# agrif/unnamed-rust-sdr

Measured on AMD Instinct MI355X. Metric: complex Msamples/sec through 255-tap FIR, 1/2/4/8 MI355X; % HBM roofline, higher is better.
Workload: dtype f32

## Files before the change

### unnamed-rust-sdr_amd/csrc/fir_mxh.hip

```cpp
#include <algorithm>
#include <climits>
#include <cstdlib>
#include <type_traits>
#include <utility>

#include "fir_kernels.hpp"

namespace sdrgpu {

namespace {

typedef _Float16 f16x8 __attribute__((ext_vector_type(8)));
typedef unsigned u32x4 __attribute__((ext_vector_type(4)));
typedef float f32x4 __attribute__((ext_vector_type(4)));

constexpr int kWaves = 8;
constexpr int kBlock = 64 * kWaves;
constexpr int kCs1 = 4;
constexpr int kCs2 = 2;
constexpr int cs_of(int D) { return D == 1 ? kCs1 : (D == 2 ? kCs2 : 1); }
constexpr int kRunTiles = 2;
constexpr int kRunTilesU8 = 8;
constexpr int kStagePerChunk = 4;
constexpr int kNonFinite = 1 << 16;

template <int NCH, int D = 4, int CS = 1>
struct GeoH {
    static constexpr int TO = 256 * CS;
    static constexpr int TI = TO * D;
    static constexpr int HR = 32 * NCH - 16 * D;
    static constexpr int H = (HR + 127) / 128 * 128;
    static constexpr int OFF = H - HR;
    static constexpr int R = H + 2 * TI;
    static constexpr int PLB = 2 * R;
    static constexpr int WODD = 2 * TI;
    static constexpr int WAVE = 4 * PLB;
    static constexpr int NG = TI / 128;
    static constexpr int NH = H / 128;
    static_assert(HR > 0 && (D == 1 || ((D == 4 || D == 2) && OFF == 0)), "geometry");
    static_assert(TI >= H && (D == 1 || TI % 1024 == 0), "ring");
    static_assert(kWaves * WAVE <= 160 * 1024, "LDS");
};

struct MxhParams {
    const float2* in;
    const unsigned* in_u8;
    long ld_in, n_in;
    const float2* hist;
    float2* hist_next;
    const float2* dummy;
    long n_out;
    int K;
    int delta;
    int sh;
    const float* taps;
    const u32x4* frags;
    float2* out;
    long ld_out;
    long tpc, spc, seg_tiles, units;
    int ftiles;
    int oblk;
    int vec_out;
    int blocked;
};

__device__ __forceinline__ f32x4 mfma(const u32x4& a, const u32x4& b, f32x4 c) {
    return __builtin_amdgcn_mfma_f32_16x16x32_f16(__builtin_bit_cast(f16x8, a),
                                                  __builtin_bit_cast(f16x8, b), c, 0, 0, 0);
}

__device__ __forceinline__ unsigned pk_rtz(float a, float b) {
    return __builtin_bit_cast(unsigned, __builtin_amdgcn_cvt_pkrtz(a, b));
}

__device__ __forceinline__ float lo_f(unsigned u) {
    return (float)__builtin_bit_cast(_Float16, (unsigned short)(u & 0xffffu));
}
__device__ __forceinline__ float hi_f(unsigned u) {
    return (float)__builtin_bit_cast(_Float16, (unsigned short)(u >> 16));
}

__device__ __forceinline__ void split2(float a, float b, unsigned& hi, unsigned& lo) {
    hi = pk_rtz(a, b);
    lo = pk_rtz(a - lo_f(hi), b - hi_f(hi));
}

__device__ __forceinline__ int sigma(int v) {
    return v < 4 ? 2 * v : (v >= 12 ? 2 * v - 16 : 2 * v - 7);
}

__device__ __forceinline__ float2 fetch1(const float2* in, const float2* hist, long j, long n_in,
                                         int K) {
    const bool inb = (j >= 0) & (j < n_in);
    const bool inh = (j < 0) & (j >= -(long)(K - 1));
    const float2 xa = in[inb ? j : 0];
    const float2 xb = hist[inh ? j + (K - 1) : 0];
    return inb ? xa : (inh ? xb : make_float2(0.f, 0.f));
}

__device__ __forceinline__ float4 fetch_pair(const float2* in, const float2* hist, long j,
                                             long n_in, int K) {
    const float2 a = fetch1(in, hist, j, n_in, K), b = fetch1(in, hist, j + 1, n_in, K);
    return make_float4(a.x, a.y, b.x, b.y);
}

__device__ __forceinline__ float2 u8_iq(unsigned short w) {
    return make_float2(((float)(w & 0xffu) - 128.0f) / 128.0f, ((float)(w >> 8) - 128.0f) / 128.0f);
}
__device__ __forceinline__ unsigned iq_u8(float2 v) {
    return (unsigned)(v.x * 128.0f + 128.0f) | ((unsigned)(v.y * 128.0f + 128.0f) << 8);
}
__device__ __forceinline__ unsigned fetch_pair_u8(const unsigned short* in, const float2* hist,
                                                  long j, long n_in, int K) {
    unsigned w = 0;
#pragma unroll
    for (int e = 0; e < 2; ++e) {
        const long q = j + e;
        const bool inb = (q >= 0) & (q < n_in);
        const bool inh = (q < 0) & (q >= -(long)(K - 1));
        const unsigned a = in[inb ? q : 0];
        const unsigned b = iq_u8(hist[inh ? q + (K - 1) : 0]);
        w |= (inb ? a : (inh ? b : 0x8080u)) << (16 * e);
    }
    return w;
}
template <int PLB>
__device__ __forceinline__ void put_pair_u8(char* lds, int a, unsigned w) {
    const float r0 = (float)(w & 0xffu) - 128.f, i0 = (float)((w >> 8) & 0xffu) - 128.f;
    const float r1 = (float)((w >> 16) & 0xffu) - 128.f, i1 = (float)(w >> 24) - 128.f;
    *reinterpret_cast<unsigned*>(lds + a) = pk_rtz(r0, r1);
    *reinterpret_cast<unsigned*>(lds + a + 2 * PLB) = pk_rtz(i0, i1);
}

__device__ __forceinline__ void st32(char* lds, int a, unsigned v) {
    *reinterpret_cast<unsigned*>(lds + a) = v;
}

template <int PLB>
__device__ __forceinline__ void put_pair(char* lds, int a, const float4& f, float sc) {
    unsigned h, l;
    split2(f.x * sc, f.z * sc, h, l);
    st32(lds, a, h);
    st32(lds, a + PLB, l);
    split2(f.y * sc, f.w * sc, h, l);
    st32(lds, a + 2 * PLB, h);
    st32(lds, a + 3 * PLB, l);
}

__device__ __forceinline__ float absmax4(float m, const float4& f) {
    auto mx = [](float a, float b) { return __builtin_elementwise_maximum(a, b); };
    return mx(mx(mx(mx(m, fabsf(f.x)), fabsf(f.y)), fabsf(f.z)), fabsf(f.w));
}

template <int CTRL>
__device__ __forceinline__ unsigned dpp_umax(unsigned x) {
    const unsigned y = (unsigned)__builtin_amdgcn_mov_dpp((int)x, CTRL, 0xf, 0xf, true);
    return x > y ? x : y;
}
__device__ __forceinline__ int wave_scale(float m) {
    unsigned x = __float_as_uint(m);
    x = dpp_umax<0xB1>(x);
    x = dpp_umax<0x4E>(x);
    x = dpp_umax<0x141>(x);
    x = dpp_umax<0x140>(x);
    const unsigned a = __builtin_amdgcn_readlane(x, 0), b = __builtin_amdgcn_readlane(x, 16);
    const unsigned c = __builtin_amdgcn_readlane(x, 32), d = __builtin_amdgcn_readlane(x, 48);
    const unsigned ab = a > b ? a : b, cd = c > d ? c : d;
    const int e = (int)((ab > cd ? ab : cd) >> 23);
    const int s = 141 - e;
    return e == 255 ? kNonFinite : (s < -126 ? -126 : (s > 126 ? 126 : s));
}

__device__ __forceinline__ float mul_add_vop2(float acc, float x, float h) {
    float p, r;
    asm("v_mul_f32 %0, %1, %2" : "=v"(p) : "v"(x), "v"(h));
    asm("v_add_f32 %0, %1, %2" : "=v"(r) : "v"(acc), "v"(p));
    return r;
}

template <int D, int CS>
__device__ __forceinline__ void exact_tile(const MxhParams& p, long ch, int tile, int sv, int g) {
#pragma clang fp contract(off)
    const int K = p.K;
    const float2* __restrict__ in = p.in + ch * p.ld_in;
    const float2* __restrict__ hist = p.hist + ch * (long)(K - 1);
    float2* __restrict__ out = p.out + ch * p.ld_out;
    const long i0 = D - 1 - p.delta;
#pragma unroll 1
    for (int o = 0; o < 4 * CS; ++o) {
        {
            const long m = (long)tile * (256 * CS) + 256 * (o >> 2) + 16 * sv + 4 * g + (o & 3);
            if (m >= p.n_out) continue;
            const long gi = i0 + (long)D * m;
            float ar = 0.f, ai = 0.f;
            if (gi - (K - 1) >= 0 && gi < p.n_in) {
                const float2* __restrict__ xp = in + gi;
                const int kb = K & ~15;
#pragma unroll 1
                for (int k = 0; k < kb; k += 16) {
                    float2 xv[16];
                    float hk[16];
#pragma unroll
                    for (int u = 0; u < 16; ++u) {
                        xv[u] = xp[-(k + u)];
                        hk[u] = p.taps[k + u];
                    }
#pragma unroll
                    for (int u = 0; u < 16; ++u) {
                        ar = mul_add_vop2(ar, xv[u].x, hk[u]);
                        ai = mul_add_vop2(ai, xv[u].y, hk[u]);
                    }
                }
#pragma unroll 1
                for (int k = kb; k < K; ++k) {
                    const float2 xv = xp[-k];
                    const float hk = p.taps[k];
                    ar = mul_add_vop2(ar, xv.x, hk);
                    ai = mul_add_vop2(ai, xv.y, hk);
                }
            } else {
#pragma unroll 1
                for (int k = 0; k < K; ++k) {
                    const float2 xv = fetch1(in, hist, gi - k, p.n_in, K);
                    const float hk = p.taps[k];
                    ar = mul_add_vop2(ar, xv.x, hk);
                    ai = mul_add_vop2(ai, xv.y, hk);
                }
            }
            out[m] = make_float2(ar, ai);
        }
    }
}

__device__ __forceinline__ float exp2i(int s) { return __builtin_amdgcn_ldexpf(1.0f, s); }

template <int NCH, int D>
__global__ __launch_bounds__(64) void tap_frag_kernel(const float* __restrict__ taps, int K, int sh,
                                                      u32x4* __restrict__ tab) {
    constexpr int HR = GeoH<NCH, D, cs_of(D)>::HR;
    const int lane = threadIdx.x, delta = blockIdx.x;
    const int g = lane >> 4, v = lane & 15;
    const float tsc = exp2i(sh);
    u32x4* __restrict__ th = tab + (size_t)delta * (2 * NCH * 64);
#pragma unroll
    for (int c = 0; c < NCH; ++c) {
        u32x4 ah, al;
#pragma unroll
        for (int jj = 0; jj < 4; ++jj) {
            unsigned hw = 0, lw = 0;
#pragma unroll
            for (int e = 0; e < 2; ++e) {
                const int pidx = 32 * c + 8 * g + 2 * jj + e;
                const int k = D * v + D - 1 - delta + HR - pidx;
                const bool ok = (k >= 0) & (k < K);
                const float hk = taps[ok ? k : 0];
                const float hs = ok ? hk * tsc : 0.f;
                const _Float16 h16 = (_Float16)hs;
                const _Float16 l16 = (_Float16)(hs - (float)h16);
                hw |= (unsigned)__builtin_bit_cast(unsigned short, h16) << (16 * e);
                lw |= (unsigned)__builtin_bit_cast(unsigned short, l16) << (16 * e);
            }
            ah[jj] = hw;
            al[jj] = lw;
        }
        th[c * 64 + lane] = ah;
        th[(NCH + c) * 64 + lane] = al;
    }
}

template <int NCH, bool U8 = false, int D = 4, int CS = 1>
__global__ __launch_bounds__(kBlock) __attribute__((amdgpu_waves_per_eu(2, 2)))
void fir_mxh_kernel(MxhParams p) {
    using Raw = std::conditional_t<U8, unsigned, float4>;
    using G = GeoH<NCH, D, CS>;
    constexpr int H = G::H, PLB = G::PLB, NH = G::NH, NG = G::NG;
    constexpr int TI = G::TI;
    extern __shared__ __attribute__((aligned(16))) char smem[];

    claim_simd_half();
    const int lane = threadIdx.x & 63;
    const int wv = __builtin_amdgcn_readfirstlane(threadIdx.x >> 6);
    if (wv >= kWaves / 2) __builtin_amdgcn_s_setprio(1);
    const long wave = (long)blockIdx.x * kWaves + wv;
    const long nwaves = (long)gridDim.x * kWaves;
    const int g = lane >> 4, v = lane & 15;
    const int K = p.K;
    const int base = wv * G::WAVE;

    u32x4 ah[NCH], al[NCH];
    const int sv = D == 4 ? sigma(v) : v;
    int rb[NCH];
    int wb0;
    auto ramp_setup = [&]() {
#pragma unroll
        for (int c = 0; c < NCH; ++c) {
            ah[c] = p.frags[c * 64 + lane];
            al[c] = p.frags[(NCH + c) * 64 + lane];
        }
#pragma unroll
        for (int c = 0; c < NCH; ++c) {
            if constexpr (D == 4) {
                const int r = sv + (c >> 1);
                rb[c] = base + 128 * r + 16 * ((4 * (c & 1) + g) ^ ((r >> 1) & 7));
            } else if constexpr (D == 2) {
                const int r = v + c;
                rb[c] = base + 64 * r + 16 * (g ^ ((r >> 1) & 3));
            } else {
                rb[c] = base + 2 * (G::OFF + 16 * sv + 32 * c + 8 * g);
            }
        }
        wb0 = D == 4   ? base + 128 * (lane >> 5) + 4 * (lane & 3) + 16 * ((lane >> 2) & 7)
              : D == 2 ? base + 64 * (lane >> 4) + 4 * (lane & 3) + 16 * (((lane >> 2) & 3) ^ (lane >> 5))
                       : base + 4 * lane;
    };

    struct Cur {
        int u, t, ch, tu, nt;
        int ok;
    };
    const int units = (int)p.units, spc = (int)p.spc, segt = (int)p.seg_tiles, tpc = (int)p.tpc;
    const int ust = p.blocked ? kWaves : (int)nwaves;
    const int ub1 = p.blocked ? (int)(((long)blockIdx.x + 1) * p.units / gridDim.x) : units;
    auto seek = [&](Cur& c, int u) {
        c.u = u;
        c.t = 0;
        c.ok = u < ub1;
        if constexpr (D == 4 && !U8) {
            c.ch = c.ok && spc < units ? u / spc : 0;
        } else {
            c.ch = c.ok ? u / spc : 0;
        }
        c.tu = (u - c.ch * spc) * segt;
        c.nt = c.ok ? std::min(segt, tpc - c.tu) : 0;
        if (c.ok && c.nt <= 0) c.ok = false;
    };
    auto adv = [&](Cur& c) {
        if (!c.ok) return;
        if (++c.t >= c.nt) seek(c, c.u + ust);
    };
    const long n_in = p.n_in;
    auto tile_j0 = [&](const Cur& c) { return (long)TI * (c.tu + c.t); };
    auto tile_fast = [&](const Cur& c) { return c.tu + c.t < p.ftiles; };
    auto fetch = [&](const Cur& c, long j) -> Raw {
        const float2* hist = p.hist + c.ch * (long)(K - 1);
        if constexpr (U8)
            return fetch_pair_u8(reinterpret_cast<const unsigned short*>(p.in_u8) + c.ch * p.ld_in, hist, j,
                                 n_in, K);
        else
            return fetch_pair(p.in + c.ch * p.ld_in, hist, j, n_in, K);
    };
    auto put = [&](int a, const Raw& w, float sc) {
        if constexpr (U8) put_pair_u8<PLB>(smem, a, w);
        else put_pair<PLB>(smem, a, w, sc);
    };
    auto ldx = [&](const Cur& c, long j, auto nt_c) -> Raw {
        constexpr bool NT = decltype(nt_c)::value;
        if constexpr (U8) {
            const unsigned* q = p.in_u8 + c.ch * (p.ld_in / 2) + (j >> 1);
            return NT ? __builtin_nontemporal_load(q) : *q;
        } else {
            const f32x4* q = reinterpret_cast<const f32x4*>(p.in + c.ch * p.ld_in + j);
            const f32x4 r = NT ? __builtin_nontemporal_load(q) : *q;
            return make_float4(r[0], r[1], r[2], r[3]);
        }
    };
    auto load_tile = [&](Raw (&dst)[NG], const Cur& c) {
        const long j0 = tile_j0(c);
        if (tile_fast(c)) {
#pragma unroll
            for (int k = 0; k < NG; ++k) dst[k] = ldx(c, j0 + 128 * k + 2 * lane, std::true_type());
        } else {
            asm volatile("" ::: "memory");
#pragma unroll
            for (int k = 0; k < NG; ++k) dst[k] = fetch(c, j0 + 128 * k + 2 * lane);
        }
    };
    auto load_hist = [&](Raw (&dst)[NH], const Cur& c) {
        const long j = tile_j0(c) - H;
        const int tile = c.tu + c.t;
        if (tile >= 1 && tile <= p.ftiles) {
#pragma unroll
            for (int k = 0; k < NH; ++k) dst[k] = ldx(c, j + 128 * k + 2 * lane, std::false_type());
        } else {
            asm volatile("" ::: "memory");
#pragma unroll
            for (int k = 0; k < NH; ++k) dst[k] = fetch(c, j + 128 * k + 2 * lane);
        }
    };
    auto window_scale = [&](const Raw (&nx)[NG], const Raw (&hr)[NH]) -> int {
        if constexpr (U8) {
            return 7;
        } else {
            float m = 0.f;
#pragma unroll
            for (int k = 0; k < NG; ++k) m = absmax4(m, nx[k]);
#pragma unroll
            for (int k = 0; k < NH; ++k) m = absmax4(m, hr[k]);
            return wave_scale(m);
        }
    };
    auto hist_addr = [&](int k) {
        if constexpr (D == 4) return (wb0 ^ (16 * (k & 7))) + 256 * k;
        else if constexpr (D == 2) return (wb0 ^ (32 * (k & 1))) + 256 * k;
        else return wb0 + 256 * k;
    };
    auto new_addr = [&](int k) {
        if constexpr (D == 4) return (wb0 ^ (16 * ((H / 128 + k) & 7))) + 128 * (H / 64 + 2 * k);
        else if constexpr (D == 2) return (wb0 ^ (32 * ((H / 128 + k) & 1))) + 2 * H + 256 * k;
        else return wb0 + 2 * H + 256 * k;
    };
    auto roll_hist = [&](Raw (&hr)[NH], const Raw (&tile)[NG]) {
        Raw nh[NH];
#pragma unroll
        for (int i = 0; i < NH; ++i) nh[i] = NG + i < NH ? hr[(NG + i) % NH] : tile[(NG + i - NH) % NG];
#pragma unroll
        for (int i = 0; i < NH; ++i) hr[i] = nh[i];
    };

    const bool ev = (v & 1) == 0;
    const unsigned om = 8u * (16 * sv + 4 * g), omp = 8u * (16 * (D == 4 ? sigma(v ^ 1) : (v ^ 1)) + 4 * g);
    const unsigned ob1 = ev ? om : omp + 16, ob2 = ev ? omp : om + 16;

    static_assert(NG <= 8 && 2 * NG > 8, "one raw tile in flight");
    static_assert(NG > NH, "an even window's last NH groups come from keep[]");
    Cur cm, st, ld;
    const int first_unit = p.blocked ? (int)((long)blockIdx.x * p.units / gridDim.x) + wv : (int)wave;
    int nf_tiles = 0;
    seek(cm, first_unit);
    if (cm.ok) {
        Raw nx[NG], hr[NH];
        load_hist(hr, cm);
        load_tile(nx, cm);
        ramp_setup();
        st = cm;
        adv(st);
        const bool st_run = st.ok && st.t == 0;
        int s_cur = window_scale(nx, hr);
        {
            const float sc = exp2i(s_cur);
#pragma unroll
            for (int k = 0; k < NH; ++k) put(hist_addr(k), hr[k], sc);
            if (st.ok && tile_fast(st)) {
                if (st_run) load_hist(hr, st);
                const long j1 = tile_j0(st);
                Raw keep[NH];
#pragma unroll
                for (int k = 0; k < NG; ++k) {
                    put(new_addr(k), nx[k], sc);
                    if (k >= NG - NH) keep[k - (NG - NH)] = nx[k];
                    nx[k] = ldx(st, j1 + 128 * k + 2 * lane, std::true_type());
                }
                if (!st_run) {
                    Raw tile[NG];
#pragma unroll
                    for (int k = 0; k < NG; ++k) tile[k] = keep[k < NG - NH ? 0 : k - (NG - NH)];
                    roll_hist(hr, tile);
                }
            } else {
#pragma unroll
                for (int k = 0; k < NG; ++k) put(new_addr(k), nx[k], sc);
                if (st_run) load_hist(hr, st);
                else roll_hist(hr, nx);
                if (st.ok) load_tile(nx, st);
            }
        }
        ld = st;
        adv(ld);

        auto body = [&](auto tau_c) {
            constexpr int TAU = decltype(tau_c)::value;
            constexpr int P = 1 - TAU;
            constexpr int WN = P * G::WODD;
            const bool fast2 = ld.ok && tile_fast(ld);
            const bool ld_run = ld.ok && ld.t == 0;
            const long j2 = tile_j0(ld);
            const float2* src2 = fast2 ? p.in + ld.ch * p.ld_in + j2 : p.dummy;
            const unsigned* src2u = fast2 ? p.in_u8 + ld.ch * (p.ld_in / 2) + (j2 >> 1)
                                          : reinterpret_cast<const unsigned*>(p.dummy);
            const int s_fresh = window_scale(nx, hr);
            const int dsc = s_fresh - s_cur;
            const bool keep_scale = P == 1 && st.t > 0 && dsc >= -1 && dsc <= 7;
            const int s_next = keep_scale ? s_cur : s_fresh;
            const bool hist_late = P == 1 && !keep_scale;
            const float scn = exp2i(s_next);
            constexpr int NK = NG < NH ? NG : NH;
            Raw keep[NK];
            f32x4 cr[CS], ci[CS];
#pragma unroll
            for (int j = 0; j < CS; ++j) {
                cr[j] = f32x4{0.f, 0.f, 0.f, 0.f};
                ci[j] = f32x4{0.f, 0.f, 0.f, 0.f};
            }
            u32x4 fb[2][4];
            auto read_frags = [&](u32x4 (&f)[4], int c, int j) {
                const int a = rb[c] + TAU * G::WODD + j * 2 * 256 * D;
#pragma unroll
                for (int q = 0; q < 4; ++q)
                    if (!U8 || (q & 1) == 0)
                        f[q] = *reinterpret_cast<const u32x4*>(smem + a + q * PLB);
            };
            read_frags(fb[0], 0, 0);
            constexpr bool kShare = D == 1 && 32 * (NCH - 1) == 256;
#pragma unroll
            for (int i = 0; i < CS * NCH; ++i) {
                const int j = i / NCH, c = i % NCH;
                {
                    const int ni = i + 1;
                    const bool reuse = kShare && ni % NCH == 0;
                    if (ni < CS * NCH && !reuse)
                        read_frags(fb[(kShare ? ni - ni / NCH : ni) & 1], ni % NCH, ni / NCH);
                    __builtin_amdgcn_sched_barrier(0);
                    const u32x4(&f)[4] = fb[(kShare ? i - j : i) & 1];
                    cr[j] = mfma(al[c], f[0], cr[j]);
                    ci[j] = mfma(al[c], f[2], ci[j]);
                    if (!U8) {
                        cr[j] = mfma(ah[c], f[1], cr[j]);
                        ci[j] = mfma(ah[c], f[3], ci[j]);
                    }
                    cr[j] = mfma(ah[c], f[0], cr[j]);
                    ci[j] = mfma(ah[c], f[2], ci[j]);
                }
                if (i == 0) {
                    if (P == 0) {
#pragma unroll
                        for (int k = 0; k < NH; ++k) put(WN + hist_addr(k), hr[k], scn);
                    }
                    if (ld_run && !hist_late) load_hist(hr, ld);
                }
#pragma unroll
                for (int k = 0; k < NG; ++k) {
                    if ((k / kStagePerChunk < CS * NCH - 1 ? k / kStagePerChunk : CS * NCH - 1) != i) continue;
                    if (P == 1 || k < NG - NH) put(WN + new_addr(k), nx[k], scn);
                    if (k >= NG - NH) keep[k - (NG > NH ? NG - NH : 0)] = nx[k];
                    if constexpr (U8) {
                        nx[k] = __builtin_nontemporal_load(src2u + 64 * k + lane);
                    } else {
                        const f32x4 r = __builtin_nontemporal_load(
                            reinterpret_cast<const f32x4*>(src2 + 128 * k + 2 * lane));
                        nx[k] = make_float4(r[0], r[1], r[2], r[3]);
                    }
                }
            }
            if constexpr (P == 0) {
#pragma unroll
                for (int k = NG - NH; k < NG; ++k) put(WN + new_addr(k), keep[k - (NG - NH)], scn);
            } else {
                if (hist_late) {
#pragma unroll
                    for (int k = 0; k < NH; ++k) put(WN + hist_addr(k), hr[k], scn);
                    if (ld_run) load_hist(hr, ld);
                }
            }
            if (!ld_run) {
                Raw tile[NG];
#pragma unroll
                for (int k = 0; k < NG; ++k) tile[k] = keep[k < (NG > NH ? NG - NH : 0) ? 0 : k - (NG > NH ? NG - NH : 0)];
                roll_hist(hr, tile);
            }
            if (!fast2 && ld.ok) load_tile(nx, ld);
            const int so = -(s_cur + p.sh);
            const int tile = cm.tu + cm.t;
            if (!U8 && s_cur == kNonFinite) {
                ++nf_tiles;
            } else {
                float2* __restrict__ out = p.out + cm.ch * p.ld_out;
                char* __restrict__ outt = reinterpret_cast<char*>(out + (long)tile * G::TO);
#pragma unroll
                for (int j = 0; j < CS; ++j) {
                    float yr[4], yi[4];
#pragma unroll
                    for (int i = 0; i < 4; ++i) {
                        yr[i] = __builtin_amdgcn_ldexpf(cr[j][i], so);
                        yi[i] = __builtin_amdgcn_ldexpf(ci[j][i], so);
                    }
                    if (p.vec_out && tile * CS + j < p.oblk) {
                        const f32x4 y0 = {yr[0], yi[0], yr[1], yi[1]};
                        const f32x4 y1 = {yr[2], yi[2], yr[3], yi[3]};
                        f32x4 rx;
#pragma unroll
                        for (int q = 0; q < 4; ++q)
                            rx[q] = __int_as_float(__builtin_amdgcn_mov_dpp(
                                __float_as_int(ev ? y1[q] : y0[q]), 0xB1, 0xf, 0xf, false));
                        __builtin_nontemporal_store(ev ? y0 : rx, reinterpret_cast<f32x4*>(outt + (ob1 + 2048u * j)));
                        __builtin_nontemporal_store(ev ? rx : y1, reinterpret_cast<f32x4*>(outt + (ob2 + 2048u * j)));
                    } else {
                        const long m = (long)tile * G::TO + 256 * j + 16 * sv + 4 * g;
#pragma unroll
                        for (int i = 0; i < 4; ++i)
                            if (m + i < p.n_out) out[m + i] = make_float2(yr[i], yi[i]);
                    }
                }
            }
            s_cur = s_next;
            cm = st;
            st = ld;
            adv(ld);
        };
        while (cm.ok) {
            body(std::integral_constant<int, 0>());
            if (!cm.ok) break;
            body(std::integral_constant<int, 1>());
        }
    }
    if constexpr (!U8) {
        if (nf_tiles > 0) {
            Cur c;
            seek(c, first_unit);
            while (c.ok) {
                const long j0 = tile_j0(c) - H;
                bool bad = false;
                for (int q = lane; q < H + TI; q += 64) {
                    const float2 xv = fetch1(p.in + c.ch * p.ld_in, p.hist + c.ch * (long)(K - 1),
                                             j0 + q, n_in, K);
                    bad |= !(__builtin_isfinite(xv.x) && __builtin_isfinite(xv.y));
                }
                if (__builtin_amdgcn_ballot_w64(bad) != 0) exact_tile<D, CS>(p, c.ch, c.tu + c.t, sv, g);
                adv(c);
            }
        }
    }

    if (p.hist_next) {
        const long nch = p.units / p.spc;
        for (long j = (long)blockIdx.x * kBlock + threadIdx.x; j < nch * (K - 1);
             j += (long)gridDim.x * kBlock) {
            const long ch = j / (K - 1), jj = j - ch * (K - 1);
            const float2* inc = p.in + ch * p.ld_in;
            const float2* hic = p.hist + ch * (long)(K - 1);
            const long gidx = p.n_in - (long)(K - 1) + jj;
            if constexpr (U8) {
                const unsigned short* inb = reinterpret_cast<const unsigned short*>(p.in_u8) + ch * p.ld_in;
                p.hist_next[j] = gidx >= 0 ? u8_iq(inb[gidx]) : hic[gidx + (K - 1)];
            } else {
                p.hist_next[j] = gidx >= 0 ? inc[gidx] : hic[gidx + (K - 1)];
            }
        }
    }
}

int mxh_nch(int K, int D) {
    if (D == 4) {
        const int need = (K + 63 + 31) / 32;
        return need <= 6 ? 6 : (need <= 10 ? 10 : 0);
    }
    if (D == 1) {
        const int need = (K + 15 + 31) / 32;
        return need <= 5 ? 5 : (need <= 9 ? 9 : 0);
    }
    if (D == 2) {
        const int need = (K + 31 + 31) / 32;
        return need <= 5 ? 5 : (need <= 9 ? 9 : 0);
    }
    return 0;
}

}

size_t fir_mxh_dummy_bytes() { return 1024 * sizeof(float2); }

int fir_mxh_shape_ok(int sample_kind, int tap_kind, int K, int D) {
    if (tap_kind != SDRGPU_F32 || K < 1) return 0;
    if (sample_kind == SDRGPU_CU8) return D == 4 && mxh_nch(K, 4) > 0;
    return sample_kind == SDRGPU_C64 && mxh_nch(K, D) > 0;
}

int fir_mxh_supported(const FirParams& fp) {
    const bool u8 = fp.sample_kind == SDRGPU_CU8;
    if ((!u8 && fp.sample_kind != SDRGPU_C64) || fp.tap_kind != SDRGPU_F32) return 0;
    if (!(fp.D == 4 || ((fp.D == 1 || fp.D == 2) && !u8))) return 0;
    if (fp.K < 1 || mxh_nch(fp.K, fp.D) == 0) return 0;
    if (fp.i0 < 0 || fp.i0 >= fp.D) return 0;
    const uintptr_t align = u8 ? 3 : 15;
    if ((reinterpret_cast<uintptr_t>(fp.in) & align) != 0 || (fp.nch > 1 && (fp.ld_in & 1)))
        return 0;
    return 1;
}

size_t fir_mxh_frag_bytes(int K, int D) {
    const int NCH = K >= 1 ? mxh_nch(K, D) : 0;
    return (size_t)D * 2 * NCH * 64 * sizeof(u32x4);
}

int fir_mxh_frag_build(const float* d_taps, int K, int D, int tap_scale_exp, void* d_frags,
                       hipStream_t s) {
    const int NCH = K >= 1 ? mxh_nch(K, D) : 0;
    if (NCH == 0 || !d_taps || !d_frags) return SDRGPU_ERR_UNSUPPORTED;
#define SDRGPU_MXH_FRAGS(CC, DD)                                                               \
    if (D == DD && NCH == CC) {                                                                \
        hipLaunchKernelGGL((tap_frag_kernel<CC, DD>), dim3(DD), dim3(64), 0, s, d_taps, K,     \
                           tap_scale_exp, static_cast<u32x4*>(d_frags));                       \
        SDRGPU_LAUNCH_CHECK();                                                                 \
        return SDRGPU_OK;                                                                      \
    }
    SDRGPU_MXH_FRAGS(10, 4)
    SDRGPU_MXH_FRAGS(6, 4)
    SDRGPU_MXH_FRAGS(9, 1)
    SDRGPU_MXH_FRAGS(5, 1)
    SDRGPU_MXH_FRAGS(9, 2)
    SDRGPU_MXH_FRAGS(5, 2)
#undef SDRGPU_MXH_FRAGS
    return SDRGPU_ERR_UNSUPPORTED;
}

int fir_mxh_launch(const FirParams& fp, const float* d_taps, int tap_scale_exp,
                   const void* d_frags, const void* d_dummy, int cus, hipStream_t s) {
    if (!fir_mxh_supported(fp) || !d_dummy || !d_frags) return SDRGPU_ERR_UNSUPPORTED;
    const int D = fp.D;
    const int NCH = mxh_nch(fp.K, D);
    MxhParams p;
    const bool u8 = fp.sample_kind == SDRGPU_CU8;
    p.in = static_cast<const float2*>(fp.in);
    p.in_u8 = static_cast<const unsigned*>(fp.in);
    p.ld_in = fp.ld_in;
    p.n_in = fp.n_in;
    p.hist = static_cast<const float2*>(fp.hist);
    p.hist_next = fp.K > 1 ? static_cast<float2*>(fp.hist_next) : nullptr;
    p.dummy = static_cast<const float2*>(d_dummy);
    p.n_out = fp.n_out;
    p.K = fp.K;
    p.delta = (int)(D - 1 - fp.i0);
    p.sh = tap_scale_exp;
    p.taps = d_taps;
    p.frags = static_cast<const u32x4*>(d_frags) + (size_t)p.delta * (2 * NCH * 64);
    p.out = static_cast<float2*>(fp.out);
    p.ld_out = fp.ld_out;
    p.vec_out = ((reinterpret_cast<uintptr_t>(fp.out) & 15) == 0 &&
                 (fp.nch == 1 || !(fp.ld_out & 1)))
                    ? 1
                    : 0;
    const long nch = fp.nch;
    const int cs = cs_of(D);
    p.tpc = ceil_div(std::max(0L, fp.n_out), 256L * cs);
    const long W = (long)kWaves * cus;
    const int run = D == 4 ? (u8 ? kRunTilesU8 : kRunTiles) : (D == 2 ? kRunTiles : 0);
    long spc = nch >= W ? 1 : ceil_div(W, nch);
    spc = std::max(1L, std::min(spc, p.tpc));
    p.seg_tiles = std::max(1L, ceil_div(p.tpc, spc));
    if (run > 0) p.seg_tiles = std::max(1L, std::min<long>(run, p.tpc));
    p.spc = std::max(1L, ceil_div(p.tpc, p.seg_tiles));
    p.units = nch * p.spc;
    p.blocked = run > 0 && u8;
    const long TI = 256L * cs * D;
    p.ftiles = (int)std::min<long>(fp.n_in / TI, INT_MAX);
    p.oblk = (int)std::min<long>(std::max(0L, fp.n_out) / 256, INT_MAX);
    if (p.units >= INT_MAX - 8L * cus || p.tpc >= INT_MAX) return SDRGPU_ERR_UNSUPPORTED;
    const long blocks = std::max(1L, std::min((long)cus, ceil_div(p.units, kWaves)));
#define SDRGPU_MXH_GO(CC, U, DD, CS)                                                           \
    hipLaunchKernelGGL((fir_mxh_kernel<CC, U, DD, CS>), dim3(blocks), dim3(kBlock),            \
                       (size_t)kWaves * (GeoH<CC, DD, CS>::WAVE), s, p)
#define SDRGPU_MXH_CASE(CC)                                                                    \
    if (D == 4 && NCH == CC) {                                                                 \
        if (u8) SDRGPU_MXH_GO(CC, true, 4, 1);                                                 \
        else SDRGPU_MXH_GO(CC, false, 4, 1);                                                   \
        SDRGPU_LAUNCH_CHECK();                                                                 \
        return SDRGPU_OK;                                                                      \
    }
#define SDRGPU_MXH_CASE1(CC)                                                                   \
    if (D == 1 && NCH == CC) {                                                                 \
        SDRGPU_MXH_GO(CC, false, 1, kCs1);                                                     \
        SDRGPU_LAUNCH_CHECK();                                                                 \
        return SDRGPU_OK;                                                                      \
    }
#define SDRGPU_MXH_CASE2(CC)                                                                   \
    if (D == 2 && NCH == CC) {                                                                 \
        SDRGPU_MXH_GO(CC, false, 2, kCs2);                                                     \
        SDRGPU_LAUNCH_CHECK();                                                                 \
        return SDRGPU_OK;                                                                      \
    }
    SDRGPU_MXH_CASE(10)
    SDRGPU_MXH_CASE(6)
    SDRGPU_MXH_CASE1(9)
    SDRGPU_MXH_CASE1(5)
    SDRGPU_MXH_CASE2(9)
    SDRGPU_MXH_CASE2(5)
#undef SDRGPU_MXH_CASE
#undef SDRGPU_MXH_CASE1
#undef SDRGPU_MXH_CASE2
#undef SDRGPU_MXH_GO
    return SDRGPU_ERR_UNSUPPORTED;
}

}
```

Before: 631,200.

## Pair real/imag columns in MFMA fragments to halve LDS fragment reads

For float input with decimation 4 or 1, the kernel now has half the lanes read real-plane and half read imag-plane fragments. Each fragment read of two registers then feeds both the real and the (shifted) imaginary accumulators, and staging is interleaved into the new chunk loop. An extra IMO pad offsets the imaginary planes in LDS to avoid bank conflicts. Outputs are re-paired with a DPP row shuffle before the vector stores. This is meant to cut LDS read traffic, at the cost of more MFMA iterations (NCH+PSH chunks), extra select and DPP work in the epilogue, and more complex indexing.

```diff
diff --git a/unnamed-rust-sdr_amd/csrc/fir_mxh.hip b/unnamed-rust-sdr_amd/csrc/fir_mxh.hip
--- a/unnamed-rust-sdr_amd/csrc/fir_mxh.hip
+++ b/unnamed-rust-sdr_amd/csrc/fir_mxh.hip
@@ -24,7 +24,7 @@
 constexpr int kStagePerChunk = 4;
 constexpr int kNonFinite = 1 << 16;
 
-template <int NCH, int D = 4, int CS = 1>
+template <int NCH, int D = 4, int CS = 1, int IMO = 0>
 struct GeoH {
     static constexpr int TO = 256 * CS;
     static constexpr int TI = TO * D;
@@ -33,14 +33,21 @@
     static constexpr int OFF = H - HR;
     static constexpr int R = H + 2 * TI;
     static constexpr int PLB = 2 * R;
+    static constexpr int IMOFF = IMO;
     static constexpr int WODD = 2 * TI;
-    static constexpr int WAVE = 4 * PLB;
+    static constexpr int WAVE = 4 * PLB + IMO;
     static constexpr int NG = TI / 128;
     static constexpr int NH = H / 128;
     static_assert(HR > 0 && (D == 1 || ((D == 4 || D == 2) && OFF == 0)), "geometry");
     static_assert(TI >= H && (D == 1 || TI % 1024 == 0), "ring");
-    static_assert(kWaves * WAVE <= 160 * 1024, "LDS");
+    static_assert(kWaves * WAVE <= 160 * 1024 && IMO % 128 == 0, "LDS");
 };
+
+constexpr bool pair_cols(bool U8, int D) { return D == 4 && !U8; }
+constexpr bool pair_cols1(bool U8, int D) { return D == 1 && !U8; }
+constexpr int pair_imo(bool U8, int D) { return pair_cols(U8, D) ? 128 : 0; }
+template <int NCH, bool U8, int D, int CS>
+using GeoK = GeoH<NCH, D, CS, pair_imo(U8, D)>;
 
 struct MxhParams {
     const float2* in;
@@ -136,15 +143,15 @@
     *reinterpret_cast<unsigned*>(lds + a) = v;
 }
 
-template <int PLB>
+template <int PLB, int IMO>
 __device__ __forceinline__ void put_pair(char* lds, int a, const float4& f, float sc) {
     unsigned h, l;
     split2(f.x * sc, f.z * sc, h, l);
     st32(lds, a, h);
     st32(lds, a + PLB, l);
     split2(f.y * sc, f.w * sc, h, l);
-    st32(lds, a + 2 * PLB, h);
-    st32(lds, a + 3 * PLB, l);
+    st32(lds, a + 2 * PLB + IMO, h);
+    st32(lds, a + 3 * PLB + IMO, l);
 }
 
 __device__ __forceinline__ float absmax4(float m, const float4& f) {
@@ -272,9 +279,15 @@
 __global__ __launch_bounds__(kBlock) __attribute__((amdgpu_waves_per_eu(2, 2)))
 void fir_mxh_kernel(MxhParams p) {
     using Raw = std::conditional_t<U8, unsigned, float4>;
-    using G = GeoH<NCH, D, CS>;
+    using G = GeoK<NCH, U8, D, CS>;
     constexpr int H = G::H, PLB = G::PLB, NH = G::NH, NG = G::NG;
     constexpr int TI = G::TI;
+    constexpr bool PAIR = pair_cols(U8, D);
+    constexpr bool PAIR1 = pair_cols1(U8, D);
+    constexpr bool PAIRS = PAIR || PAIR1;
+    constexpr int PSH = PAIR ? 2 : 4;
+    constexpr int SETCH = 8;
+    constexpr int NRD = PAIR ? NCH + 2 : NCH;
     extern __shared__ __attribute__((aligned(16))) char smem[];
 
     claim_simd_half();
@@ -289,7 +302,8 @@
 
     u32x4 ah[NCH], al[NCH];
     const int sv = D == 4 ? sigma(v) : v;
-    int rb[NCH];
+    const int pw = v & 7, pim = ((v + 4) >> 3) & 1;
+    int rb[NRD];
     int wb0;
     auto ramp_setup = [&]() {
 #pragma unroll
@@ -298,8 +312,13 @@
             al[c] = p.frags[(NCH + c) * 64 + lane];
         }
 #pragma unroll
-        for (int c = 0; c < NCH; ++c) {
-            if constexpr (D == 4) {
+        for (int c = 0; c < NRD; ++c) {
+            if constexpr (PAIR) {
+                const int r = 2 * pw + (c >> 1);
+                rb[c] = base + pim * (2 * PLB + G::IMOFF) + 128 * r + 16 * ((4 * (c & 1) + g) ^ ((pw + (c >> 2)) & 7));
+            } else if constexpr (PAIR1) {
+                rb[c] = base + pim * 2 * PLB + 2 * (G::OFF + 16 * pw + 32 * c + 8 * g);
+            } else if constexpr (D == 4) {
                 const int r = sv + (c >> 1);
                 rb[c] = base + 128 * r + 16 * ((4 * (c & 1) + g) ^ ((r >> 1) & 7));
             } else if constexpr (D == 2) {
@@ -351,7 +370,7 @@
     };
     auto put = [&](int a, const Raw& w, float sc) {
         if constexpr (U8) put_pair_u8<PLB>(smem, a, w);
-        else put_pair<PLB>(smem, a, w, sc);
+        else put_pair<PLB, G::IMOFF>(smem, a, w, sc);
     };
     auto ldx = [&](const Cur& c, long j, auto nt_c) -> Raw {
         constexpr bool NT = decltype(nt_c)::value;
@@ -499,18 +518,65 @@
                     if (!U8 || (q & 1) == 0)
                         f[q] = *reinterpret_cast<const u32x4*>(smem + a + q * PLB);
             };
-            read_frags(fb[0], 0, 0);
-            constexpr bool kShare = D == 1 && 32 * (NCH - 1) == 256;
-#pragma unroll
-            for (int i = 0; i < CS * NCH; ++i) {
-                const int j = i / NCH, c = i % NCH;
-                {
+            auto read_pair = [&](u32x4 (&f)[4], int c) {
+                const int a = (PAIR1 ? rb[0] + 64 * c : rb[c]) + TAU * G::WODD;
+                f[0] = *reinterpret_cast<const u32x4*>(smem + a);
+                f[1] = *reinterpret_cast<const u32x4*>(smem + a + PLB);
+            };
+            if constexpr (PAIRS) read_pair(fb[0], 0);
+            else read_frags(fb[0], 0, 0);
+            if constexpr (PAIRS) {
+                constexpr int NIT = (CS - 1) * SETCH + NCH + PSH;
+                constexpr int NST = (NG + kStagePerChunk - 1) / kStagePerChunk;
+                static_assert(NST < NIT, "staging chunks");
+                auto stage = [&](int i) __attribute__((always_inline)) {
+                    if (i == 0) {
+                        if (P == 0) {
+#pragma unroll
+                            for (int k = 0; k < NH; ++k) put(WN + hist_addr(k), hr[k], scn);
+                        }
+                        if (ld_run && !hist_late) load_hist(hr, ld);
+                    }
+#pragma unroll
+                    for (int k = 0; k < NG; ++k) {
+                        if (k / kStagePerChunk != i) continue;
+                        if (P == 1 || k < NG - NH) put(WN + new_addr(k), nx[k], scn);
+                        if (k >= NG - NH) keep[k - (NG - NH)] = nx[k];
+                        const f32x4 r = __builtin_nontemporal_load(
+                            reinterpret_cast<const f32x4*>(src2 + 128 * k + 2 * lane));
+                        nx[k] = make_float4(r[0], r[1], r[2], r[3]);
+                    }
+                };
+                auto chunk = [&](int i) __attribute__((always_inline)) {
+                    if (i + 1 < NIT) read_pair(fb[(i + 1) & 1], i + 1);
+                    __builtin_amdgcn_sched_barrier(0);
+                    const u32x4(&f)[4] = fb[i & 1];
+#pragma unroll
+                    for (int m = 0; m < 3; ++m) {
+#pragma unroll
+                        for (int j = 0; j < CS; ++j) {
+                            const int c = i - SETCH * j;
+                            if (c >= 0 && c < NCH) cr[j] = mfma(m == 0 ? al[c] : ah[c], f[m == 1], cr[j]);
+                            if (c >= PSH && c < NCH + PSH)
+                                ci[j] = mfma(m == 0 ? al[c - PSH] : ah[c - PSH], f[m == 1], ci[j]);
+                        }
+                    }
+                };
+#pragma unroll
+                for (int i = 0; i < NST; ++i) {
+                    chunk(i);
+                    stage(i);
+                }
+#pragma unroll
+                for (int i = NST; i < NIT; ++i) chunk(i);
+            } else {
+#pragma unroll
+                for (int i = 0; i < CS * NCH; ++i) {
+                    const int j = i / NCH, c = i % NCH;
                     const int ni = i + 1;
-                    const bool reuse = kShare && ni % NCH == 0;
-                    if (ni < CS * NCH && !reuse)
-                        read_frags(fb[(kShare ? ni - ni / NCH : ni) & 1], ni % NCH, ni / NCH);
+                    if (ni < CS * NCH) read_frags(fb[ni & 1], ni % NCH, ni / NCH);
                     __builtin_amdgcn_sched_barrier(0);
-                    const u32x4(&f)[4] = fb[(kShare ? i - j : i) & 1];
+                    const u32x4(&f)[4] = fb[i & 1];
                     cr[j] = mfma(al[c], f[0], cr[j]);
                     ci[j] = mfma(al[c], f[2], ci[j]);
                     if (!U8) {
@@ -519,25 +585,25 @@
                     }
                     cr[j] = mfma(ah[c], f[0], cr[j]);
                     ci[j] = mfma(ah[c], f[2], ci[j]);
-                }
-                if (i == 0) {
-                    if (P == 0) {
-#pragma unroll
-                        for (int k = 0; k < NH; ++k) put(WN + hist_addr(k), hr[k], scn);
-                    }
-                    if (ld_run && !hist_late) load_hist(hr, ld);
-                }
-#pragma unroll
-                for (int k = 0; k < NG; ++k) {
-                    if ((k / kStagePerChunk < CS * NCH - 1 ? k / kStagePerChunk : CS * NCH - 1) != i) continue;
-                    if (P == 1 || k < NG - NH) put(WN + new_addr(k), nx[k], scn);
-                    if (k >= NG - NH) keep[k - (NG > NH ? NG - NH : 0)] = nx[k];
-                    if constexpr (U8) {
-                        nx[k] = __builtin_nontemporal_load(src2u + 64 * k + lane);
-                    } else {
-                        const f32x4 r = __builtin_nontemporal_load(
-                            reinterpret_cast<const f32x4*>(src2 + 128 * k + 2 * lane));
-                        nx[k] = make_float4(r[0], r[1], r[2], r[3]);
+                    if (i == 0) {
+                        if (P == 0) {
+#pragma unroll
+                            for (int k = 0; k < NH; ++k) put(WN + hist_addr(k), hr[k], scn);
+                        }
+                        if (ld_run && !hist_late) load_hist(hr, ld);
+                    }
+#pragma unroll
+                    for (int k = 0; k < NG; ++k) {
+                        if ((k / kStagePerChunk < CS * NCH - 1 ? k / kStagePerChunk : CS * NCH - 1) != i) continue;
+                        if (P == 1 || k < NG - NH) put(WN + new_addr(k), nx[k], scn);
+                        if (k >= NG - NH) keep[k - (NG > NH ? NG - NH : 0)] = nx[k];
+                        if constexpr (U8) {
+                            nx[k] = __builtin_nontemporal_load(src2u + 64 * k + lane);
+                        } else {
+                            const f32x4 r = __builtin_nontemporal_load(
+                                reinterpret_cast<const f32x4*>(src2 + 128 * k + 2 * lane));
+                            nx[k] = make_float4(r[0], r[1], r[2], r[3]);
+                        }
                     }
                 }
             }
@@ -565,29 +631,66 @@
             } else {
                 float2* __restrict__ out = p.out + cm.ch * p.ld_out;
                 char* __restrict__ outt = reinterpret_cast<char*>(out + (long)tile * G::TO);
-#pragma unroll
-                for (int j = 0; j < CS; ++j) {
-                    float yr[4], yi[4];
-#pragma unroll
-                    for (int i = 0; i < 4; ++i) {
-                        yr[i] = __builtin_amdgcn_ldexpf(cr[j][i], so);
-                        yi[i] = __builtin_amdgcn_ldexpf(ci[j][i], so);
-                    }
-                    if (p.vec_out && tile * CS + j < p.oblk) {
-                        const f32x4 y0 = {yr[0], yi[0], yr[1], yi[1]};
-                        const f32x4 y1 = {yr[2], yi[2], yr[3], yi[3]};
+                if constexpr (PAIRS) {
+                    constexpr unsigned PB = PAIR ? 16 : 128;
+                    const unsigned po = (PAIR ? 32 : 16) * pw + 4 * g + 2 * pim;
+#pragma unroll
+                    for (int j = 0; j < CS; ++j) {
+                        float a0[4], a1[4];
+#pragma unroll
+                        for (int i = 0; i < 4; ++i) {
+                            a0[i] = __builtin_amdgcn_ldexpf(cr[j][i], so);
+                            a1[i] = __builtin_amdgcn_ldexpf(ci[j][i], so);
+                        }
+                        const bool im = pim != 0;
+                        const f32x4 tx = {im ? a0[0] : a0[2], im ? a0[1] : a0[3], im ? a1[0] : a1[2],
+                                          im ? a1[1] : a1[3]};
                         f32x4 rx;
 #pragma unroll
                         for (int q = 0; q < 4; ++q)
-                            rx[q] = __int_as_float(__builtin_amdgcn_mov_dpp(
-                                __float_as_int(ev ? y1[q] : y0[q]), 0xB1, 0xf, 0xf, false));
-                        __builtin_nontemporal_store(ev ? y0 : rx, reinterpret_cast<f32x4*>(outt + (ob1 + 2048u * j)));
-                        __builtin_nontemporal_store(ev ? rx : y1, reinterpret_cast<f32x4*>(outt + (ob2 + 2048u * j)));
-                    } else {
-                        const long m = (long)tile * G::TO + 256 * j + 16 * sv + 4 * g;
-#pragma unroll
-                        for (int i = 0; i < 4; ++i)
-                            if (m + i < p.n_out) out[m + i] = make_float2(yr[i], yi[i]);
+                            rx[q] = __int_as_float(
+                                __builtin_amdgcn_mov_dpp(__float_as_int(tx[q]), 0x128, 0xf, 0xf, false));
+                        const f32x4 y0 = {im ? rx[0] : a0[0], im ? a0[2] : rx[0], im ? rx[1] : a0[1],
+                                          im ? a0[3] : rx[1]};
+                        const f32x4 y1 = {im ? rx[2] : a1[0], im ? a1[2] : rx[2], im ? rx[3] : a1[1],
+                                          im ? a1[3] : rx[3]};
+                        if (p.vec_out && tile * CS + j < p.oblk) {
+                            __builtin_nontemporal_store(y0, reinterpret_cast<f32x4*>(outt + (8u * po + 2048u * j)));
+                            __builtin_nontemporal_store(y1, reinterpret_cast<f32x4*>(outt + (8u * (po + PB) + 2048u * j)));
+                        } else {
+                            const long m = (long)tile * G::TO + 256 * j + po;
+#pragma unroll
+                            for (int i = 0; i < 2; ++i) {
+                                if (m + i < p.n_out) out[m + i] = make_float2(y0[2 * i], y0[2 * i + 1]);
+                                if (m + PB + i < p.n_out) out[m + PB + i] = make_float2(y1[2 * i], y1[2 * i + 1]);
+                            }
+                        }
+                    }
+                } else {
+#pragma unroll
+                    for (int j = 0; j < CS; ++j) {
+                        float yr[4], yi[4];
+#pragma unroll
+                        for (int i = 0; i < 4; ++i) {
+                            yr[i] = __builtin_amdgcn_ldexpf(cr[j][i], so);
+                            yi[i] = __builtin_amdgcn_ldexpf(ci[j][i], so);
+                        }
+                        if (p.vec_out && tile * CS + j < p.oblk) {
+                            const f32x4 y0 = {yr[0], yi[0], yr[1], yi[1]};
+                            const f32x4 y1 = {yr[2], yi[2], yr[3], yi[3]};
+                            f32x4 rx;
+#pragma unroll
+                            for (int q = 0; q < 4; ++q)
+                                rx[q] = __int_as_float(__builtin_amdgcn_mov_dpp(
+                                    __float_as_int(ev ? y1[q] : y0[q]), 0xB1, 0xf, 0xf, false));
+                            __builtin_nontemporal_store(ev ? y0 : rx, reinterpret_cast<f32x4*>(outt + (ob1 + 2048u * j)));
+                            __builtin_nontemporal_store(ev ? rx : y1, reinterpret_cast<f32x4*>(outt + (ob2 + 2048u * j)));
+                        } else {
+                            const long m = (long)tile * G::TO + 256 * j + 16 * sv + 4 * g;
+#pragma unroll
+                            for (int i = 0; i < 4; ++i)
+                                if (m + i < p.n_out) out[m + i] = make_float2(yr[i], yi[i]);
+                        }
                     }
                 }
             }
@@ -747,7 +850,7 @@
     const long blocks = std::max(1L, std::min((long)cus, ceil_div(p.units, kWaves)));
 #define SDRGPU_MXH_GO(CC, U, DD, CS)                                                           \
     hipLaunchKernelGGL((fir_mxh_kernel<CC, U, DD, CS>), dim3(blocks), dim3(kBlock),            \
-                       (size_t)kWaves * (GeoH<CC, DD, CS>::WAVE), s, p)
+                       (size_t)kWaves * (GeoK<CC, U, DD, CS>::WAVE), s, p)
 #define SDRGPU_MXH_CASE(CC)                                                                    \
     if (D == 4 && NCH == CC) {                                                                 \
         if (u8) SDRGPU_MXH_GO(CC, true, 4, 1);                                                 \
```

Result: slower. 622,300 (-1.4%).
